# helgeanl/GP-MPC

Measured on NVIDIA H100. Metric: GP predictions/sec (N train x horizon test, fp64), higher is better.
Workload: dtype f64

## Files before the change

gp-mpc_b200/csrc/gpmpc.cu:

```cuda
#include "../../include/gpmpc.h"

#include <dlfcn.h>
#include <math.h>
#include <stdarg.h>
#include <stdlib.h>
#include <string.h>

#include <algorithm>
#include <type_traits>
#include <vector>

#include <nvtx3/nvToolsExt.h>

#include "common.cuh"
#include "gemm_dmma.cuh"
#include "predict_streamk.cuh"
#include "kernels.cuh"

#define GPMPC_VERSION 100
#define HB 64
#define NX_MAX 32
#define PSK_MAX_CTAS 2048
#define MAX_DEPTH 12
#define LOOKAHEAD_MIN_ROWS 1024
// ... 29 lines not shown
        snprintf(err, errn, "libnccl is missing required symbols");
        g_nccl.lib = nullptr;
        return false;
    }
    return true;
}

template <typename T>
struct DevBuf {
    T* p = nullptr;
    size_t cap = 0;
    DevBuf() = default;
    DevBuf(const DevBuf&) = delete;
    DevBuf& operator=(const DevBuf&) = delete;
    ~DevBuf() { cudaFree(p); }
    operator T*() const { return p; }
    int ensure(gpmpc_handle_t h, long long count, const char* name);
};

struct gpmpc_handle_s {
    int N = 0, Nx = 0, Ny = 0, a0 = 0, nloc = 0, Npad = 0, device = 0;
    int nloc_max = 0;
    cudaStream_t st = nullptr;
    cudaEvent_t ev0 = nullptr, ev1 = nullptr;
    cudaStream_t sideSt[MAX_DEPTH] = {nullptr}; cudaEvent_t evA[MAX_DEPTH] = {nullptr}, evB[MAX_DEPTH] = {nullptr}, evT[MAX_DEPTH] = {nullptr}, evS[MAX_DEPTH] = {nullptr};
    long long w2off[MAX_DEPTH + 1] = {0};
    DevBuf<double> dXT, dMu, dY, dHyp, dJit, dHypTmp;
    DevBuf<double> dL, dLi, dW1, dW2;
    DevBuf<double> dAlpha, dTmp, dRes;
    DevBuf<int> dInfo;
    DevBuf<double> dKST, dPart, dPMJ, dSQ, dV, dR, dR2;
    DevBuf<unsigned int> dCnt;
    int psk_ctas = 0, opt_predict_ctas = 0;
    DevBuf<double> dCovV, dCovOut;
    DevBuf<double> dUall, dBeta, dPDV, dPH, dGradOut; bool u_valid = false;
    DevBuf<double> dDR, dVD, dPG, dPB2, dPM3, dHessOut;
    DevBuf<double> dG;
    double *dZ = nullptr, *dSigma = nullptr, *dMean = nullptr, *dVar = nullptr, *dJ = nullptr, *dCov = nullptr;
    DevBuf<double> dRoll;
    DevBuf<double> dIn, dOut;
    int Hcap = 0;
    double* hPinned = nullptr; double* dPinnedAlias = nullptr; size_t hPinnedBytes = 0;
    DevBuf<double> dU, dKinv, dGradPart, dGrad;
    bool has_data = false, has_hyper = false, factorized = false;
    DevBuf<double> dEmTr, dEMP, dEmE, dEmF, dEmW, dEmIJ;
    DevBuf<double> dEmMeanPart, dEmPart, dEmLQ, dEmVec, dEmE2, dEmF2;
    DevBuf<double> dEmKinv, dEmGPart, dEmGRec, dEmBB; bool em_kinv_valid = false;
    std::vector<double> hyper;
    std::vector<double> logdet, yalpha;
    std::vector<int> jitter_used;
    int sms = 132;
    int opt_refine = 0, opt_small_tiles = 528;
    nccl_comm_t comm = nullptr; int rank = 0, world = 1;
    DevBuf<double> dPeerBlock; long long peerGsz = 0; int peerHcap = 0; bool peer_ready = false;
    double* peerBase[GPMPC_MAXW] = {nullptr}; bool peerOpened[GPMPC_MAXW] = {false};
    int* dPeerStatus = nullptr; int* hPeerStatus = nullptr;
    unsigned long long peer_step = 0; int opt_peer = 1; double opt_peer_timeout_s = 60.0; int clock_khz = 1980000;
    char err[512] = "";
};

static void set_error(gpmpc_handle_t h, const char* fmt, ...)
{
    va_list ap; va_start(ap, fmt);
    vsnprintf(h ? h->err : g_create_err, 512, fmt, ap);
    va_end(ap);
}
// ... 198 lines not shown
        const double jit = attempt ? jitter : 0.0;
        CUDA_TRY(cudaMemcpyAsync(h->dJit + a, &jit, sizeof(double), cudaMemcpyHostToDevice, h->st));
        CUDA_TRY(cudaMemsetAsync(h->dInfo + a, 0, sizeof(int), h->st));
        {
            int rck = launch_kbuild(h, dHyp, h->dJit + a, L, 1, 0);
            if (rck) return rck;
        }
        int rc = potrf_inv_rec(h, L, Li, slab(h), slab(h), h->dInfo + a, 0, h->Npad, 1);
        if (rc) return rc;
        int info = 0;
        CUDA_TRY(cudaMemcpyAsync(&info, h->dInfo + a, sizeof(int), cudaMemcpyDeviceToHost, h->st));
        CUDA_TRY(cudaStreamSynchronize(h->st));
        if (info == 0) { *used = attempt; return GPMPC_OK; }
        *used = 1 + info;
    }
    return GPMPC_ERR_NOTPD;
}

extern "C" int gpmpc_version(void) { return GPMPC_VERSION; }

extern "C" const char* gpmpc_last_error(gpmpc_handle_t h) { return h ? h->err : g_create_err; }

extern "C" int gpmpc_destroy(gpmpc_handle_t h);

static int create_fill(gpmpc_handle_t h, int N, int Nx, int Ny, int out_begin, int out_count, int device)
{
    h->N = N; h->Nx = Nx; h->Ny = Ny; h->a0 = out_begin; h->nloc = out_count; h->device = device;
    h->nloc_max = out_count; h->world = 1; h->rank = 0;
    h->Npad = (N + GPMPC_TILE - 1) / GPMPC_TILE * GPMPC_TILE;
    CUDA_TRY(cudaSetDevice(device));
    CUDA_TRY(cudaDeviceGetAttribute(&h->sms, cudaDevAttrMultiProcessorCount, device));
    h->opt_small_tiles = 4 * h->sms;
    h->psk_ctas = PSK_CTAS_PER_SM * h->sms;
    cudaDeviceGetAttribute(&h->clock_khz, cudaDevAttrClockRate, device);
    {
        int lo = 0, hi = 0;
        cudaDeviceGetStreamPriorityRange(&lo, &hi);
        CUDA_TRY(cudaStreamCreateWithPriority(&h->st, cudaStreamNonBlocking, hi));
    }
    CUDA_TRY(cudaEventCreate(&h->ev0));
    CUDA_TRY(cudaEventCreate(&h->ev1));
    const long long np = h->Npad;
    ENSURE(h->dXT, (long long)Nx * np);
    ENSURE(h->dMu, NX_MAX);
    ENSURE(h->dY, (long long)out_count * np);
    ENSURE(h->dHyp, (long long)out_count * (Nx + 2));
    ENSURE(h->dHypTmp, Nx + 2);
    ENSURE(h->dJit, out_count);
    ENSURE(h->dL, out_count * slab(h));
    ENSURE(h->dLi, out_count * slab(h));
    {
        const int nb = h->Npad / 128;
        long long off = 0;
        for (int d = 0; d < MAX_DEPTH; ++d) {
            h->w2off[d] = off;
            const long long nd = (long long)((nb + (1 << d) - 1) >> d) * 128;
            off += nd * nd / 4 + 128;
        }
        h->w2off[MAX_DEPTH] = off;
        int lo = 0, hi = 0;
        cudaDeviceGetStreamPriorityRange(&lo, &hi);
        for (int d = 0; d < MAX_DEPTH; ++d) {
            CUDA_TRY(cudaStreamCreateWithPriority(&h->sideSt[d], cudaStreamNonBlocking, lo));
            CUDA_TRY(cudaEventCreateWithFlags(&h->evA[d], cudaEventDisableTiming));
            CUDA_TRY(cudaEventCreateWithFlags(&h->evB[d], cudaEventDisableTiming));
            CUDA_TRY(cudaEventCreateWithFlags(&h->evT[d], cudaEventDisableTiming));
// ... 291 lines not shown
    if (what == GPMPC_GET_K) return gpmpc_build_K(h, a, dst);
    if (what == GPMPC_GET_ALPHA_NLML) {
        CUDA_TRY(cudaMemcpyAsync(dst, h->dAlpha + (long long)al * h->Npad, h->N * 8, cudaMemcpyDeviceToHost, h->st));
        CUDA_TRY(cudaStreamSynchronize(h->st));
        return GPMPC_OK;
    }
    if (!h->factorized) { set_error(h, "gpmpc_get: call gpmpc_factorize first"); return GPMPC_ERR_STATE; }
    switch (what) {
    case GPMPC_GET_CHOL: return extract_to_host(h, h->dL + (long long)al * slab(h), dst, 1);
    case GPMPC_GET_LINV: return extract_to_host(h, h->dLi + (long long)al * slab(h), dst, 1);
    case GPMPC_GET_ALPHA:
        CUDA_TRY(cudaMemcpyAsync(dst, h->dAlpha + (long long)al * h->Npad, h->N * 8, cudaMemcpyDeviceToHost, h->st));
        CUDA_TRY(cudaStreamSynchronize(h->st));
        return GPMPC_OK;
    case GPMPC_GET_LOGDET: dst[0] = h->logdet[al]; return GPMPC_OK;
    case GPMPC_GET_INVK: {
        int rc = compute_kinv(h, al);
        if (rc) return rc;
        return extract_to_host(h, h->dKinv, dst, 2);
    }
    default: set_error(h, "gpmpc_get: unknown selector %d", what); return GPMPC_ERR_ARG;
    }
}

extern "C" int gpmpc_set_option(gpmpc_handle_t h, const char* name, double value)
{
    if (!h || !name) return GPMPC_ERR_ARG;
    if (!strcmp(name, "refine")) { h->opt_refine = value != 0.0; return GPMPC_OK; }
    if (!strcmp(name, "predict_ctas")) {
        const int v = (int)value;
        if (v < 0 || v > PSK_MAX_CTAS) { set_error(h, "predict_ctas must be in [0, %d]", PSK_MAX_CTAS); return GPMPC_ERR_ARG; }
        h->opt_predict_ctas = v; return GPMPC_OK;
    }
    if (!strcmp(name, "peer_timeout_s")) { h->opt_peer_timeout_s = value > 0.0 ? value : 60.0; return GPMPC_OK; }
    if (!strcmp(name, "small_tiles")) { h->opt_small_tiles = (int)value; return GPMPC_OK; }
    if (!strcmp(name, "peer")) { h->opt_peer = value != 0.0; return GPMPC_OK; }
    set_error(h, "unknown option %s", name);
    return GPMPC_ERR_ARG;
}

static inline int ks_chunk(gpmpc_handle_t h)
{
    if (h->Npad < 8192) return 128;
    return (h->nloc >= 2 && h->Nx <= 12) ? 1024 : 512;
}

static inline int ks_blocks(gpmpc_handle_t h) { return (h->Npad + ks_chunk(h) - 1) / ks_chunk(h); }

static int ensure_rows(gpmpc_handle_t h)
{
    ENSURE(h->dV, (long long)h->nloc * HB * h->Npad);
    ENSURE(h->dR, (long long)h->nloc * HB * h->Npad);
    return GPMPC_OK;
}

static int ensure_predict_bufs(gpmpc_handle_t h, int H)
{
    const long long np = h->Npad, nt = np / 128;
    ENSURE(h->dKST, (long long)h->nloc * HB * np);
    ENSURE(h->dPMJ, (long long)h->nloc * HB * ks_blocks(h) * (h->Nx + 1));
    ENSURE(h->dSQ, (long long)h->nloc * HB * nt);
    ENSURE(h->dCnt, (long long)h->nloc * nt + h->nloc + 1);
    ENSURE(h->dPart, (long long)std::max(h->psk_ctas, h->opt_predict_ctas) * 2 * HB * PSK_BN);
    if (h->opt_refine) {
        int rc = ensure_rows(h);
        if (rc) return rc;
        ENSURE(h->dR2, (long long)h->nloc * HB * np);
    }
    if (H > h->Hcap) {
        h->Hcap = 0;
        h->dZ = h->dSigma = h->dMean = h->dVar = h->dJ = h->dCov = nullptr;
        const long long cap = std::max(H, HB);
        const int nyp = h->nloc_max * h->world;
        const long long Nx = h->Nx, Ny = h->Ny;
        ENSURE(h->dG, (long long)nyp * cap * (Nx + 2));
        ENSURE(h->dIn, cap * Nx + cap * Nx * Nx);
        ENSURE(h->dOut, cap * (2 * Ny + Ny * Nx + Ny * Ny));
        h->dZ = h->dIn; h->dSigma = h->dIn + cap * Nx;
        h->dMean = h->dOut; h->dVar = h->dOut + cap * Ny; h->dJ = h->dOut + 2 * cap * Ny;
        h->dCov = h->dOut + 2 * cap * Ny + cap * Ny * Nx;
        h->Hcap = (int)cap;
    }
    return GPMPC_OK;
}

template <int BM>
static cudaError_t psk_launch_bm(const PredictParams& p, const double* A, long long sA, const double* B, long long sB,
                                 int np, int grid, cudaStream_t st)
{
    constexpr int BYTES = psk_pipe_doubles(BM) * 8 + 2 * PSK_STAGES * 8 + 1024;
    const cudaError_t e = smem_opt_in<predict_streamk_kernel<BM>>(BYTES);
    if (e != cudaSuccess) return e;
    CUtensorMap tmA, tmB;
    if (!tmap_make(&tmA, A, np, BM, np, sA, p.nloc, BM)) return cudaErrorInvalidValue;
    if (!tmap_make(&tmB, B, np, np, np, sB, p.nloc, PSK_BN)) return cudaErrorInvalidValue;
    cudaLaunchConfig_t cfg;
    memset(&cfg, 0, sizeof(cfg));
    cfg.gridDim = dim3(grid); cfg.blockDim = dim3(PSK_THREADS); cfg.dynamicSmemBytes = BYTES; cfg.stream = st;
    cudaLaunchAttribute attr[1];
    attr[0].id = cudaLaunchAttributeProgrammaticStreamSerialization;
    attr[0].val.programmaticStreamSerializationAllowed = 1;
    cfg.attrs = attr; cfg.numAttrs = 1;
    return cudaLaunchKernelEx(&cfg, predict_streamk_kernel<BM>, p, tmA, tmB);
}

static cudaError_t psk_launch(int bm, const PredictParams& p, const double* A, long long sA, const double* B, long long sB,
                              int np, int grid, cudaStream_t st)
{
    switch (bm) {
    case 8: return psk_launch_bm<8>(p, A, sA, B, sB, np, grid, st);
    case 16: return psk_launch_bm<16>(p, A, sA, B, sB, np, grid, st);
    case 24: return psk_launch_bm<24>(p, A, sA, B, sB, np, grid, st);
    case 32: return psk_launch_bm<32>(p, A, sA, B, sB, np, grid, st);
    case 40: return psk_launch_bm<40>(p, A, sA, B, sB, np, grid, st);
    case 48: return psk_launch_bm<48>(p, A, sA, B, sB, np, grid, st);
    case 56: return psk_launch_bm<56>(p, A, sA, B, sB, np, grid, st);
    default: return psk_launch_bm<64>(p, A, sA, B, sB, np, grid, st);
    }
}

static int psk_grid(gpmpc_handle_t h, long long G)
{
    int ctas = h->opt_predict_ctas > 0 ? h->opt_predict_ctas : h->psk_ctas;
    ctas = std::min(ctas, PSK_MAX_CTAS);
    const long long by_work = std::max(1LL, G / 4);
    return (int)std::min<long long>(ctas, h->opt_predict_ctas > 0 ? G : by_work);
}

static void psk_base(gpmpc_handle_t h, PredictParams& p, int Hc, int upper = 0)
{
    memset(&p, 0, sizeof(p));
    const long long nt = h->Npad / 128;
    p.nloc = h->nloc; p.nt = (int)nt; p.Hc = Hc; p.upper = upper;
    p.ntb = (int)((h->Npad + PSK_BN - 1) / PSK_BN); p.nk = h->Npad / GEMM_BK;
    p.T = psk_steps_per_output(p.ntb, p.nk, upper); p.G = p.T * h->nloc;
    p.part = h->dPart;
    p.tile_cnt = h->dCnt; p.out_cnt = h->dCnt + (long long)h->nloc * nt; p.done_cnt = p.out_cnt + h->nloc;
    p.SQ = h->dSQ;
    p.hyp = h->dHyp; p.hyp_ld = h->Nx + 2; p.Nx = h->Nx;
}

static void psk_finalize(gpmpc_handle_t h, PredictParams& p, int H, int h0)
{
    p.finalize = 1; p.PMJ = h->dPMJ; p.nblk_mj = ks_blocks(h);
    p.Gloc = h->dG; p.slot0 = h->a0; p.Htot = H; p.h0 = h0;
}

static AssembleArgs assemble_args(gpmpc_handle_t h, int H, int method, const double* Sigma, int spp,
                                  double* mean, double* var, double* J, double* cov)
{
    AssembleArgs as;
    memset(&as, 0, sizeof(as));
    as.G = h->dG; as.Ny = h->Ny; as.Nx = h->Nx; as.H = H; as.method_ta = (method == GPMPC_METHOD_TA);
    as.Sigma = Sigma; as.sigma_per_point = spp;
    as.mean = mean; as.var = var; as.J = J; as.cov = cov;
    as.world = 1;
    const long long bm1 = (std::min(H, HB) + 7) / 8 * 8;
    as.stage_g = (assemble_rows_doubles(H, h->Ny, h->Nx) <= psk_pipe_doubles((int)bm1)) ? 1 : 0;
    return as;
}

template <int NXP, int CH>
static cudaError_t launch_ks(gpmpc_handle_t h, const double* dZc, int Hc, int bm, int nblk)
{
    const int smem = (NXP + 1) * CH * 8;
    const cudaError_t e = smem_opt_in<ks_tile_kernel<NXP, CH>>(smem);
    if (e != cudaSuccess) return e;
    dim3 g(nblk, bm / 8, h->nloc);
// ... 4 lines not shown

template <int CH>
static cudaError_t launch_ks_nx(gpmpc_handle_t h, const double* dZc, int Hc, int bm, int nblk)
{
    const int Nx = h->Nx;
    if (Nx <= 4) return launch_ks<4, CH>(h, dZc, Hc, bm, nblk);
    if (Nx <= 6) return launch_ks<6, CH>(h, dZc, Hc, bm, nblk);
    if (Nx <= 8) return launch_ks<8, CH>(h, dZc, Hc, bm, nblk);
    if (Nx <= 10) return launch_ks<10, CH>(h, dZc, Hc, bm, nblk);
    if (Nx <= 12) return launch_ks<12, CH>(h, dZc, Hc, bm, nblk);
    if (CH <= 512) {
        if (Nx <= 16) return launch_ks<16, (CH <= 512 ? CH : 512)>(h, dZc, Hc, bm, nblk);
        if (Nx <= 24) return launch_ks<24, (CH <= 512 ? CH : 512)>(h, dZc, Hc, bm, nblk);
        return launch_ks<32, (CH <= 512 ? CH : 512)>(h, dZc, Hc, bm, nblk);
    }
    return cudaErrorInvalidValue;
}

static cudaError_t launch_ks_any(gpmpc_handle_t h, const double* dZc, int Hc, int bm, int nblk)
{
    switch (ks_chunk(h)) {
    case 1024: return launch_ks_nx<1024>(h, dZc, Hc, bm, nblk);
    case 512: return launch_ks_nx<512>(h, dZc, Hc, bm, nblk);
    default: return launch_ks_nx<128>(h, dZc, Hc, bm, nblk);
    }
}

static int tri_product(gpmpc_handle_t h, const double* Amat, const double* T, int bm, int Hc, double* Vout)
{
    const int np = h->Npad;
    PredictParams p;
    psk_base(h, p, Hc);
    p.Vout = Vout; p.sV = (long long)HB * np; p.ldv = np;
    CUDA_TRY(psk_launch(bm, p, Amat, (long long)HB * np, T, slab(h), np, psk_grid(h, p.G), h->st));
    return GPMPC_OK;
}

__global__ void axpby_rows_kernel(const double* __restrict__ x, const double* __restrict__ y, double a, double b,
                                  double* __restrict__ out, long long rowlen, long long srow, int rows)
{
    const long long i = (long long)blockIdx.x * blockDim.x + threadIdx.x;
    const int r = blockIdx.y, bz = blockIdx.z;
    if (i >= rowlen || r >= rows) return;
    const long long o = (long long)bz * srow + (long long)r * rowlen + i;
    out[o] = a * x[o] + b * y[o];
}

static int predict_core(gpmpc_handle_t h, int method, int H, const double* dZ, const double* dSigma, int spp,
                        double* d_mean, double* d_var, double* d_cov, double* d_jac)
{
    const int np = h->Npad, Nx = h->Nx;
    NvtxRange nvtx_r("gpmpc.predict");
    const int use_peers = (h->world > 1 && h->peer_ready && h->opt_peer && H <= h->peerHcap) ? 1 : 0;
    const int nccl_gather = (h->world > 1 && !use_peers) ? 1 : 0;
    const long long timeout_clocks = (long long)(h->opt_peer_timeout_s * 1e3 * (double)h->clock_khz);
    PeerArgs pa;
    memset(&pa, 0, sizeof(pa));
    if (use_peers) {
        h->peer_step += 1;
        for (int r = 0; r < h->world; ++r) pa.base[r] = h->peerBase[r];
        pa.world = h->world; pa.rank = h->rank;
        pa.goff = 2 * GPMPC_MAXW + (long long)(h->peer_step & 1) * h->peerGsz;
        pa.flag_idx = (int)(h->peer_step & 1) * GPMPC_MAXW + h->rank;
        pa.step = h->peer_step;
        pa.timeout_clocks = timeout_clocks;
    }
    AssembleArgs as = assemble_args(h, H, method, dSigma, spp, d_mean, d_var, d_jac, d_cov);
    if (use_peers) as.G = h->dPeerBlock + pa.goff;
    as.flags = use_peers ? reinterpret_cast<const unsigned long long*>(h->dPeerBlock.p) + (h->peer_step & 1) * GPMPC_MAXW : nullptr;
    as.world = h->world; as.step = h->peer_step; as.status = h->dPeerStatus; as.timeout_clocks = timeout_clocks;
    const bool fused_assemble = (H <= HB) && !nccl_gather && ((long long)H * h->Ny * Nx * 8 <= 64 * 1024);
    for (int h0 = 0; h0 < H; h0 += HB) {
        const int Hc = std::min(HB, H - h0);
        const int bm = (Hc + 7) / 8 * 8;
        const bool last_chunk = (h0 + HB >= H);
        const double* dZc = dZ + (long long)h0 * Nx;
        CUDA_TRY(launch_ks_any(h, dZc, Hc, bm, ks_blocks(h)));
        PredictParams p;
        psk_base(h, p, Hc);
        psk_finalize(h, p, H, h0);
        p.pa = pa; p.use_peers = use_peers; p.publish = last_chunk ? 1 : 0;
        p.as = as; p.do_assemble = (fused_assemble && !h->opt_refine) ? 1 : 0;
        if (!h->opt_refine) {
            CUDA_TRY(psk_launch(bm, p, h->dKST, (long long)HB * np, h->dLi, slab(h), np, psk_grid(h, p.G), h->st));
        } else {
            int rc = tri_product(h, h->dKST, h->dLi, bm, Hc, h->dV);
            if (rc) return rc;
            rc = tri_product(h, h->dV, h->dL, bm, Hc, h->dR);
            if (rc) return rc;
            dim3 g((np + 255) / 256, bm, h->nloc);
            axpby_rows_kernel<<<g, 256, 0, h->st>>>(h->dKST, h->dR, 1.0, -1.0, h->dR, np, (long long)HB * np, bm);
            CUDA_TRY(cudaGetLastError());
            rc = tri_product(h, h->dR, h->dLi, bm, Hc, h->dR2);
            if (rc) return rc;
            axpby_rows_kernel<<<g, 256, 0, h->st>>>(h->dV, h->dR2, 1.0, 1.0, h->dV, np, (long long)HB * np, bm);
            CUDA_TRY(cudaGetLastError());
            sq_rows_kernel<<<dim3(np / 128, Hc, h->nloc), 128, 0, h->st>>>(h->dV, np, (long long)HB * np, h->dSQ, np / 128);
            CUDA_TRY(cudaGetLastError());
            finalize_kernel<<<h->nloc, PSK_THREADS, 0, h->st>>>(p);
            CUDA_TRY(cudaGetLastError());
        }
    }
    if (nccl_gather) {
        const size_t cnt = (size_t)h->nloc_max * H * (Nx + 2);
        int r = g_nccl.AllGather(h->dG + (size_t)h->rank * cnt, h->dG, cnt, 8 , h->comm, h->st);
        if (r) { set_error(h, "ncclAllGather failed: %s", g_nccl.GetErrorString ? g_nccl.GetErrorString(r) : "?"); return GPMPC_ERR_NCCL; }
    }
    if (!fused_assemble || h->opt_refine) {
        const int smem = (2 * h->Ny * Nx + h->Ny) * 8;
        assemble_kernel<<<std::min(H, 2048), 128, smem, h->st>>>(as);
        CUDA_TRY(cudaGetLastError());
    }
    return GPMPC_OK;
}

static bool lu_factor(int n, double* A, int* piv, double* det)
{
// ... 643 lines not shown
    }
    const long long per = (long long)Ny * Nx + (long long)Ny * Ny * Nx + (long long)Ny * Nx * Nx;
    ENSURE(h->dGradOut, (long long)std::max(H, HB) * per);
    double* d_dvar = h->dGradOut;
    double* d_dcov = d_dvar + (long long)H * Ny * Nx;
    double* d_hess = d_dcov + (long long)H * Ny * Ny * Nx;
    const long long nxx = (long long)Nx * Nx, ntri = (long long)Nx * (Nx + 1) * (Nx + 2) / 6;
    double *d_d2var = nullptr, *d_d3mean = nullptr, *d_d2cov = nullptr, *d_sh = nullptr;
    if (ho) {
        ENSURE(h->dDR, (long long)h->nloc * HB * np);
        ENSURE(h->dVD, (long long)h->nloc * HB * np);
        ENSURE(h->dPG, (long long)h->nloc * HB * nblk_g * npairs);
        ENSURE(h->dPB2, (long long)h->nloc * HB * nblk_g * npairs);
        ENSURE(h->dPM3, (long long)h->nloc * HB * nblk_g * ntri);
        const long long hper = 2 * Ny * nxx + Ny * nxx * Nx + (long long)Ny * Ny * nxx;
        ENSURE(h->dHessOut, (long long)std::max(H, HB) * hper);
        d_d2var = h->dHessOut;
        d_sh = d_d2var + (long long)H * Ny * nxx;
        d_d3mean = d_sh + (long long)H * Ny * nxx;
        d_d2cov = d_d3mean + (long long)H * Ny * nxx * Nx;
    }
    const size_t nz = (size_t)H * Nx, ns = (method == GPMPC_METHOD_TA) ? (size_t)(spp ? H : 1) * Nx * Nx : 0;
    CUDA_TRY(cudaMemcpyAsync(h->dZ, Z, nz * 8, cudaMemcpyHostToDevice, h->st));
    if (ns) CUDA_TRY(cudaMemcpyAsync(h->dSigma, Sigma, ns * 8, cudaMemcpyHostToDevice, h->st));
    const AssembleArgs as = assemble_args(h, H, method, h->dSigma, spp, h->dMean, h->dVar, h->dJ, h->dCov);
    for (int h0 = 0; h0 < H; h0 += HB) {
        const int Hc = std::min(HB, H - h0), bm = (Hc + 7) / 8 * 8;
        const double* dZc = h->dZ + (long long)h0 * Nx;
        CUDA_TRY(launch_ks_any(h, dZc, Hc, bm, ks_blocks(h)));
        PredictParams p;
        psk_base(h, p, Hc);
        psk_finalize(h, p, H, h0);
        p.Vout = h->dV; p.sV = (long long)HB * np; p.ldv = np;
        CUDA_TRY(psk_launch(bm, p, h->dKST, (long long)HB * np, h->dLi, slab(h), np, psk_grid(h, p.G), h->st));
        psk_base(h, p, Hc, 1);
        p.Vout = h->dBeta; p.sV = (long long)HB * np; p.ldv = np;
        CUDA_TRY(psk_launch(bm, p, h->dV, (long long)HB * np, h->dUall, slab(h), np, psk_grid(h, p.G), h->st));
        CUDA_TRY(nxp_dispatch(Nx, [&](auto nxp) { return launch_grad_reduce<decltype(nxp)::value>(h, dZc, Hc, nblk_g); }));
        grad_finalize_kernel<<<dim3(Hc, h->nloc), 128, 0, h->st>>>(h->dPDV, h->dPH, nblk_g, Hc, h->dHyp, Nx + 2, Nx, Ny,
                                                                   h->dG, H, h0, d_dvar, d_hess);
        CUDA_TRY(cudaGetLastError());
        if (ho) {
            rc = hess_chunk(h, dZc, Hc, H, h0, d_d2var, d_d3mean);
            if (rc) return rc;
        }
    }
    {
        const int smem = (2 * Ny * Nx + Ny) * 8;
        assemble_kernel<<<std::min(H, 2048), 128, smem, h->st>>>(as);
        CUDA_TRY(cudaGetLastError());
        grad_cov_kernel<<<H, 128, 2 * Ny * Nx * 8, h->st>>>(Ny, Nx, method == GPMPC_METHOD_TA, h->dSigma, spp, h->dJ, d_dvar, d_hess, d_dcov);
        CUDA_TRY(cudaGetLastError());
        if (ho) {
            hess_cov_kernel<<<H, 128, 2 * Ny * Nx * 8, h->st>>>(Ny, Nx, method == GPMPC_METHOD_TA, h->dSigma, spp, h->dJ, d_hess,
                                                                d_d2var, d_d3mean, d_sh, d_d2cov);
            CUDA_TRY(cudaGetLastError());
        }
    }
    if (mean) CUDA_TRY(cudaMemcpyAsync(mean, h->dMean, (size_t)H * Ny * 8, cudaMemcpyDeviceToHost, h->st));
    if (var) CUDA_TRY(cudaMemcpyAsync(var, h->dVar, (size_t)H * Ny * 8, cudaMemcpyDeviceToHost, h->st));
    if (cov) CUDA_TRY(cudaMemcpyAsync(cov, h->dCov, (size_t)H * Ny * Ny * 8, cudaMemcpyDeviceToHost, h->st));
    if (jac) CUDA_TRY(cudaMemcpyAsync(jac, h->dJ, (size_t)H * Ny * Nx * 8, cudaMemcpyDeviceToHost, h->st));
    if (dvar_dz) CUDA_TRY(cudaMemcpyAsync(dvar_dz, d_dvar, (size_t)H * Ny * Nx * 8, cudaMemcpyDeviceToHost, h->st));
    if (dcov_dz) CUDA_TRY(cudaMemcpyAsync(dcov_dz, d_dcov, (size_t)H * Ny * Ny * Nx * 8, cudaMemcpyDeviceToHost, h->st));
    if (hess) CUDA_TRY(cudaMemcpyAsync(hess, d_hess, (size_t)H * Ny * Nx * Nx * 8, cudaMemcpyDeviceToHost, h->st));
    if (ho && ho->d2var_dz2) CUDA_TRY(cudaMemcpyAsync(ho->d2var_dz2, d_d2var, (size_t)H * Ny * nxx * 8, cudaMemcpyDeviceToHost, h->st));
    if (ho && ho->d3mean_dz3) CUDA_TRY(cudaMemcpyAsync(ho->d3mean_dz3, d_d3mean, (size_t)H * Ny * nxx * Nx * 8, cudaMemcpyDeviceToHost, h->st));
    if (ho && ho->d2cov_dz2) CUDA_TRY(cudaMemcpyAsync(ho->d2cov_dz2, d_d2cov, (size_t)H * Ny * Ny * nxx * 8, cudaMemcpyDeviceToHost, h->st));
    CUDA_TRY(cudaStreamSynchronize(h->st));
    return GPMPC_OK;
// ... 181 lines not shown
    }
    h->peer_ready = true; h->peer_step = 0;
    return GPMPC_OK;
}

extern "C" int gpmpc_get_size(gpmpc_handle_t h, int* N, int* Nx, int* Ny)
{
    if (!h) return GPMPC_ERR_ARG;
    if (N) *N = h->N;
    if (Nx) *Nx = h->Nx;
    if (Ny) *Ny = h->Ny;
    return GPMPC_OK;
}

extern "C" void* gpmpc_stream(gpmpc_handle_t h) { return h ? (void*)h->st : nullptr; }

extern "C" int gpmpc_synchronize(gpmpc_handle_t h)
{
    if (!h) return GPMPC_ERR_ARG;
    CUDA_TRY(cudaSetDevice(h->device));
    CUDA_TRY(cudaStreamSynchronize(h->st));
    return peer_status_check(h);
}

extern "C" int gpmpc_profile_balance(gpmpc_handle_t h, int H, double* out4)
{
    if (!h || !out4 || H < 1 || H > HB) return GPMPC_ERR_ARG;
    if (!h->factorized) { set_error(h, "gpmpc_profile_balance: call gpmpc_factorize first"); return GPMPC_ERR_STATE; }
    CUDA_TRY(cudaSetDevice(h->device));
    int rc = ensure_predict_bufs(h, HB);
    if (rc) return rc;
    PredictParams p;
    psk_base(h, p, H);
    const int grid = psk_grid(h, p.G);
    DevBuf<unsigned long long> dbg;
    ENSURE(dbg, (long long)grid * 2);
    p.dbg = dbg;
    const int np = h->Npad, bm = (H + 7) / 8 * 8;
    for (int rep = 0; rep < 2; ++rep) {
        cudaError_t e = psk_launch(bm, p, h->dKST, (long long)HB * np, h->dLi, slab(h), np, grid, h->st);
        if (e != cudaSuccess) { set_error(h, "profile_balance: %s", cudaGetErrorString(e)); return GPMPC_ERR_CUDA; }
    }
    std::vector<unsigned long long> t((size_t)grid * 2);
    cudaMemcpyAsync(t.data(), dbg, t.size() * 8, cudaMemcpyDeviceToHost, h->st);
    cudaStreamSynchronize(h->st);
    unsigned long long lo = ~0ull, hi = 0; double mn = 1e300, mx = 0.0, sum = 0.0;
    for (int c = 0; c < grid; ++c) {
        const double d = (double)(t[2 * c + 1] - t[2 * c]) * 1e-3;
        mn = std::min(mn, d); mx = std::max(mx, d); sum += d;
        lo = std::min(lo, t[2 * c]); hi = std::max(hi, t[2 * c + 1]);
    }
    out4[0] = mn; out4[1] = mx; out4[2] = sum / grid; out4[3] = (double)(hi - lo) * 1e-3;
    return GPMPC_OK;
}

extern "C" int gpmpc_profile_tail(gpmpc_handle_t h, int H, double* out8)
{
    if (!h || !out8 || H < 1 || H > HB) return GPMPC_ERR_ARG;
    if (!h->factorized) { set_error(h, "gpmpc_profile_tail: call gpmpc_factorize first"); return GPMPC_ERR_STATE; }
    if (h->world != 1 || h->nloc != h->Ny) { set_error(h, "gpmpc_profile_tail: single-rank handles only"); return GPMPC_ERR_STATE; }
    CUDA_TRY(cudaSetDevice(h->device));
    int rc = ensure_predict_bufs(h, HB);
    if (rc) return rc;
    const int np = h->Npad, bm = (H + 7) / 8 * 8;
    PredictParams p;
    psk_base(h, p, H);
    const int grid = psk_grid(h, p.G);
    DevBuf<unsigned long long> dbg;
    ENSURE(dbg, (long long)grid * 2 + 8);
    p.dbg = dbg;
    psk_finalize(h, p, H, 0);
    p.as = assemble_args(h, H, GPMPC_METHOD_TA, h->dSigma, 0, h->dMean, h->dVar, h->dJ, h->dCov);
    p.as.dbg = dbg + 2 * grid;
    p.do_assemble = 1;
    for (int rep = 0; rep < 2; ++rep) {
        cudaError_t e = psk_launch(bm, p, h->dKST, (long long)HB * np, h->dLi, slab(h), np, grid, h->st);
        if (e != cudaSuccess) { set_error(h, "profile_tail: %s", cudaGetErrorString(e)); return GPMPC_ERR_CUDA; }
    }
    std::vector<unsigned long long> t((size_t)grid * 2 + 8);
    cudaMemcpyAsync(t.data(), dbg, t.size() * 8, cudaMemcpyDeviceToHost, h->st);
    cudaStreamSynchronize(h->st);
    unsigned long long lo = ~0ull, hi = 0, hi2 = 0; int cmax = 0;
    for (int c = 0; c < grid; ++c) {
        lo = std::min(lo, t[2 * c]);
        if (t[2 * c + 1] > hi) { hi2 = hi; hi = t[2 * c + 1]; cmax = c; } else hi2 = std::max(hi2, t[2 * c + 1]);
    }
    for (int k = 0; k < 6; ++k) out8[k] = ((double)t[2 * grid + k] - (double)hi2) * 1e-3;
    out8[6] = (double)(hi - lo) * 1e-3;
    out8[7] = (double)(t[2 * cmax + 1] - t[2 * cmax]) * 1e-3;
    return GPMPC_OK;
}

extern "C" int gpmpc_profile_leaf(gpmpc_handle_t h, double* out15)
{
    if (!h || !out15) return GPMPC_ERR_ARG;
    if (!h->has_data || !h->has_hyper) { set_error(h, "gpmpc_profile_leaf: set_data and set_hyper first"); return GPMPC_ERR_STATE; }
    CUDA_TRY(cudaSetDevice(h->device));
    DevBuf<long long> d;
    ENSURE(d, 16);
    CUDA_TRY(cudaMemcpyToSymbol(d_leaf_prof, &d.p, sizeof(d.p)));
// ... 29 lines not shown
            const int n1 = (nn / 128 / 2) * 128, n2 = nn - n1;
            if (n1 < 128) { set_error(h, "gpmpc_profile: SYRK needs N >= 256"); return GPMPC_ERR_ARG; }
            GemmParams p;
            memset(&p, 0, sizeof(p));
            p.A = h->dW1; p.lda = n1; p.B = h->dW1; p.ldb = n1;
            p.C = h->dLi; p.ldc = np; p.Cin = h->dLi; p.ldcin = np;
            p.mt = n2 / 128; p.nt = n2 / 128; p.K = n1; p.alpha = -1e-30; p.beta = 1.0; p.lower = 1;
            cudaError_t e = gemm128(h, h->st, true, p, 1);
            if (e != cudaSuccess) { set_error(h, "profile syrk: %s", cudaGetErrorString(e)); return GPMPC_ERR_CUDA; }
            return GPMPC_OK;
        }
        case GPMPC_PROF_FACTORIZE: {
            int r = launch_kbuild(h, h->dHyp, h->dJit, h->dL, 1, 0);
            if (r) return r;
            return potrf_inv_rec(h, h->dL, h->dLi, slab(h), slab(h), h->dInfo, 0, np, 1);
        }
        case GPMPC_PROF_TRIGEMM: {
            const int Hc = (n > 0 && n <= HB) ? n : 56;
            return tri_product(h, h->dKST, h->dLi, (Hc + 7) / 8 * 8, Hc, nullptr);
        }
        case GPMPC_PROF_KS: {
            const int Hc = (n > 0 && n <= HB) ? n : 56;
            cudaError_t e = launch_ks_any(h, h->dZ, Hc, (Hc + 7) / 8 * 8, ks_blocks(h));
            if (e != cudaSuccess) { set_error(h, "profile ks: %s", cudaGetErrorString(e)); return GPMPC_ERR_CUDA; }
            return GPMPC_OK;
        }
        case GPMPC_PROF_PREDICT_TAIL: {
            const int Hc = (n > 0 && n <= HB) ? n : 56;
            PredictParams p;
            psk_base(h, p, Hc);
            psk_finalize(h, p, Hc, 0);
            p.as = assemble_args(h, Hc, GPMPC_METHOD_TA, h->dSigma, 0, h->dMean, h->dVar, h->dJ, h->dCov);
            p.do_assemble = (h->world == 1 && h->nloc == h->Ny) ? 1 : 0;
            cudaError_t e = psk_launch((Hc + 7) / 8 * 8, p, h->dKST, (long long)HB * np, h->dLi, slab(h), np, psk_grid(h, p.G), h->st);
            if (e != cudaSuccess) { set_error(h, "profile predict tail: %s", cudaGetErrorString(e)); return GPMPC_ERR_CUDA; }
            return GPMPC_OK;
        }
        default: set_error(h, "gpmpc_profile: unknown selector %d", what); return GPMPC_ERR_ARG;
        }
    };
    if (what == GPMPC_PROF_TRIGEMM || what == GPMPC_PROF_KS || what == GPMPC_PROF_PREDICT_TAIL) { rc = ensure_predict_bufs(h, HB); if (rc) return rc; }
    CUDA_TRY(cudaMemsetAsync(h->dJit, 0, h->nloc * sizeof(double), h->st));
    rc = run();
    if (rc) return rc;
    CUDA_TRY(cudaStreamSynchronize(h->st));
    CUDA_TRY(cudaEventRecord(h->ev0, h->st));
    for (int r = 0; r < reps; ++r) { rc = run(); if (rc) return rc; }
    CUDA_TRY(cudaEventRecord(h->ev1, h->st));
    CUDA_TRY(cudaEventSynchronize(h->ev1));
    CUDA_TRY(cudaEventElapsedTime(&ms, h->ev0, h->ev1));
    ms_out[0] = (double)ms / reps;
    if (what != GPMPC_PROF_TRIGEMM && what != GPMPC_PROF_KS && what != GPMPC_PROF_PREDICT_TAIL) h->factorized = false;
    return GPMPC_OK;
}
```

gp-mpc_b200/csrc/predict_streamk.cuh:

```cuda
#pragma once
#include "common.cuh"
#include "gemm_dmma.cuh"

#define GPMPC_MAXW 16
#define PSK_CW 8
#define PSK_BN (32 * PSK_CW)
#define PSK_STAGES 5
#define PSK_CTAS_PER_SM 1
#define PSK_THREADS (32 * PSK_CW)

__host__ __device__ constexpr long long psk_pipe_doubles(int bm) { return (long long)PSK_STAGES * (bm + PSK_BN) * GEMM_BK; }


struct PeerArgs {
    double* base[GPMPC_MAXW];
    int world, rank;
    long long goff;
    int flag_idx;
    unsigned long long step;
    long long timeout_clocks;
};

struct AssembleArgs {
    const double* G;
    int Ny, Nx, H, method_ta;
    const double* Sigma; int sigma_per_point;
    double *mean, *var, *J, *cov;
    const unsigned long long* flags;
    int world; unsigned long long step; int* status;
    long long timeout_clocks;
    unsigned long long* dbg;
    int stage_g;
};

struct PredictParams {
    int nloc, nt, Hc;
    int ntb, nk;
    int upper;
    long long T, G;
    double* part;
    unsigned int* tile_cnt;
    unsigned int* out_cnt;
    unsigned int* done_cnt;
    double* SQ;
    double* Vout; long long sV; int ldv;
    int finalize;
    const double* PMJ; int nblk_mj;
    const double* hyp; int hyp_ld, Nx;
    double* Gloc; int slot0, Htot, h0;
    PeerArgs pa; int use_peers, publish;
    AssembleArgs as; int do_assemble;
    unsigned long long* dbg;
};

__device__ __forceinline__ void tail_stamp(unsigned long long* dbg, int k, int tid)
{
    if (dbg && tid == 0) { unsigned long long t; asm volatile("mov.u64 %0, %%globaltimer;" : "=l"(t)); dbg[k] = t; }
}

template <bool WARP>
__device__ __forceinline__ void assemble_point(const AssembleArgs& A, int h, double* sh, int tid, int nth)
{
    const int Ny = A.Ny, Nx = A.Nx, H = A.H;
    double* Jh = sh; double* JS = sh + Ny * Nx; double* vh = sh + 2 * Ny * Nx;
    for (int idx = tid; idx < Ny * Nx; idx += nth) {
        const int a = idx / Nx, d = idx % Nx;
        const double v = __ldcg(A.G + (((long long)a) * H + h) * (Nx + 2) + 2 + d);
        Jh[idx] = v;
        if (A.J) A.J[((long long)h * Ny + a) * Nx + d] = v;
    }
    for (int a = tid; a < Ny; a += nth) {
        const double* g = A.G + (((long long)a) * H + h) * (Nx + 2);
// ... 176 lines not shown
                *reinterpret_cast<volatile int*>(A.status) = 1 + tid;
                *reinterpret_cast<volatile int*>(sh_ok) = 0;
                break;
            }
            __nanosleep(64);
        } while (true);
    }
    __syncthreads();
    return *reinterpret_cast<volatile int*>(sh_ok) != 0;
}

__global__ void __launch_bounds__(128)
assemble_kernel(const AssembleArgs A)
{
    extern __shared__ double sh[];
    __shared__ int ok;
    if (!peer_acquire(A, threadIdx.x, &ok)) return;
    for (int h = blockIdx.x; h < A.H; h += gridDim.x) assemble_point<false>(A, h, sh, threadIdx.x, blockDim.x);
}

#define PSK_SB (PSK_BN / GEMM_BK)
__host__ __device__ inline long long psk_kstart(int ntb, int nk, int upper, int jt)
{
    const long long full = (long long)(PSK_SB / 2) * jt * (jt + 1), d = (long long)PSK_SB * ntb - nk;
    return upper ? full - jt * d : (jt == ntb ? full - d : full);
}
__host__ __device__ inline long long psk_steps_per_output(int ntb, int nk, int upper) { return psk_kstart(ntb, nk, upper, ntb); }
__device__ __forceinline__ long long psk_kstart(const PredictParams& p, int jt) { return psk_kstart(p.ntb, p.nk, p.upper, jt); }
__device__ __forceinline__ int psk_ksteps(const PredictParams& p, int jt)
{
    return p.upper ? p.nk - PSK_SB * (p.ntb - 1 - jt) : min(PSK_SB * (jt + 1), p.nk);
}

struct PskIter { int a, jt, s, ks; };

__device__ __forceinline__ void psk_iter_init(PskIter& it, long long g, const PredictParams& p)
{
    it.a = (int)(g / p.T);
    const long long r = g - (long long)it.a * p.T;
    int jt = (int)((sqrt(8.0 * (double)r / PSK_SB + 1.0) - 1.0) * 0.5);
    jt = max(0, min(jt, p.ntb - 1));
    while (jt > 0 && psk_kstart(p, jt) > r) --jt;
    while (jt + 1 < p.ntb && psk_kstart(p, jt + 1) <= r) ++jt;
    it.jt = jt; it.s = (int)(r - psk_kstart(p, jt)); it.ks = psk_ksteps(p, jt);
}
__device__ __forceinline__ void psk_iter_next(PskIter& it, const PredictParams& p)
{
    if (++it.s == it.ks) {
        it.s = 0;
        if (++it.jt == p.ntb) { it.jt = 0; ++it.a; }
        it.ks = psk_ksteps(p, it.jt);
    }
}

__device__ __forceinline__ void psk_store_record(const PredictParams& p, int a, int h, int q, double val)
{
    const long long off = (((long long)(p.slot0 + a)) * p.Htot + p.h0 + h) * (p.Nx + 2) + q;
    if (!p.use_peers) p.Gloc[off] = val;
    else for (int r = 0; r < p.pa.world; ++r) p.pa.base[r][p.pa.goff + off] = val;
}

__device__ __forceinline__ void psk_reduce_mj(const PredictParams& p, int i_begin, int i_end, int t, int nthr)
{
    const int F1 = p.Nx + 1;
    for (int i = i_begin + t; i < i_end; i += nthr) {
        const int ah = i / F1, qq = i - ah * F1, a = ah / p.Hc, h = ah - a * p.Hc;
// ... 85 lines not shown
    extern __shared__ double sh[];
    __shared__ unsigned int s_flag;
    __shared__ int s_ok;
    const int per = p.Hc * (p.Nx + 1);
    psk_reduce_mj(p, blockIdx.x * per, (blockIdx.x + 1) * per, threadIdx.x, PSK_THREADS);
    psk_finalize_output(p, blockIdx.x, threadIdx.x, PSK_THREADS);
    psk_step_tail(p, sh, threadIdx.x, PSK_THREADS, &s_flag, &s_ok);
}

template <int BM>
__global__ void __launch_bounds__(PSK_THREADS, PSK_CTAS_PER_SM)
predict_streamk_kernel(const PredictParams p, const __grid_constant__ CUtensorMap tmA, const __grid_constant__ CUtensorMap tmB)
{
    constexpr int BK = GEMM_BK, BN = PSK_BN, STAGES = PSK_STAGES, CW = PSK_CW, NT = PSK_THREADS;
    constexpr int NF = BM / 8;
    static_assert(BK == 16 && BN == 32 * CW && BN % 128 == 0, "one m16n8k16 per fragment and k-step, 32 L-rows per warp");
    constexpr int GR = BN / 128;
    constexpr int A_STAGE = BM * BK, B_STAGE = BN * BK;
    constexpr uint32_t STAGE_TX = (BM + BN) * BK * 8;
    static_assert(BM % 8 == 0 && BM >= 8 && BM <= 64, "BM");

    extern __shared__ __align__(16) double smem_raw[];
    double* smem = smem_align1024(smem_raw);
    double* As = smem;
    double* Bs = smem + STAGES * A_STAGE;
    uint64_t* full = reinterpret_cast<uint64_t*>(smem + STAGES * (A_STAGE + B_STAGE));
    uint64_t* empty = full + STAGES;
    __shared__ double red[BN / 16][64];
    __shared__ unsigned int s_flag;
    __shared__ int s_ok;

    const int tid = threadIdx.x, warp = tid >> 5, lane = tid & 31, g = lane >> 2, t = lane & 3;
    const long long C = gridDim.x, c = blockIdx.x;
    const long long g0 = p.G * c / C;
    const int nsteps = (int)(p.G * (c + 1) / C - g0);
    if (nsteps <= 0) return;
    if (p.dbg && threadIdx.x == 0) { unsigned long long t0; asm volatile("mov.u64 %0, %%globaltimer;" : "=l"(t0)); p.dbg[2 * blockIdx.x] = t0; }

    __shared__ PskIter s_pit;
    __shared__ int s_pg;
    __shared__ uint64_t s_pol[2];
    if (tid == 0) {
#pragma unroll
        for (int s = 0; s < STAGES; ++s) { mbar_init(full + s, 1); mbar_init(empty + s, CW); }
        mbar_fence_init();
    }
    __syncthreads();

    auto issue = [&]() {
        PskIter it = s_pit;
        const int pg = s_pg, s = pg % STAGES;
        if (pg >= STAGES) mbar_wait(empty + s, (uint32_t)(((pg / STAGES) - 1) & 1));
        mbar_arrive_expect_tx(full + s, STAGE_TX);
        const int jta = p.upper ? p.ntb - 1 - it.jt : it.jt;
        const int k0 = (p.upper ? jta * BN : 0) + it.s * BK;
        tma_tile_g2s_3d_hint(As + s * A_STAGE, &tmA, k0, 0, it.a, full + s, s_pol[1]);
        tma_tile_g2s_3d_hint(Bs + s * B_STAGE, &tmB, k0, jta * BN, it.a, full + s, s_pol[0]);
        psk_iter_next(it, p);
        s_pit = it;
        s_pg = pg + 1;
    };
    constexpr int AHEAD = STAGES - 2;
    asm volatile("griddepcontrol.wait;" ::: "memory");
    if (tid == 0) {
        PskIter it;
        psk_iter_init(it, g0, p);
        s_pit = it; s_pg = 0;
        s_pol[0] = l2_policy_evict_first(); s_pol[1] = l2_policy_evict_last();
#pragma unroll
        for (int s = 0; s < AHEAD; ++s)
            if (s_pg < nsteps) issue();
    }
    if (p.finalize) {
        const int tot = p.nloc * p.Hc * (p.Nx + 1), per = (tot + (int)C - 1) / (int)C;
        if (tid >= 32) {
            psk_reduce_mj(p, min(tot, (int)c * per), min(tot, ((int)c + 1) * per), tid - 32, NT - 32);
            if (p.use_peers) __threadfence_system();
        }
    }

    PskIter cit;
    psk_iter_init(cit, g0, p);
    int cj[4];
#pragma unroll
    for (int j = 0; j < 4; ++j) cj[j] = (((j + 4 * (t >> 1)) ^ g) << 1) + (t & 1);
    int i = 0;
    while (i < nsteps) {
        const int a = cit.a, jt = cit.jt, s_begin = cit.s, ksteps = cit.ks;
        const int seg = min(ksteps - s_begin, nsteps - i);
        const int hh = warp / (128 / 32);
        const int st_lo = p.upper ? (128 / BK) * hh : 0;
        const int st_hi = p.upper ? ksteps : PSK_SB * jt + (128 / BK) * (hh + 1);
        double acc[2][NF][4];
#pragma unroll
        for (int mi = 0; mi < 2; ++mi)
#pragma unroll
            for (int ni = 0; ni < NF; ++ni)
#pragma unroll
                for (int r = 0; r < 4; ++r) acc[mi][ni][r] = 0.0;

        for (int q = 0; q < seg; ++q, ++i) {
            const int s = i % STAGES;
            if (tid == 0 && i + AHEAD < nsteps) issue();
            mbar_wait(full + s, (uint32_t)((i / STAGES) & 1));
            const int st = s_begin + q;
            if (st >= st_lo && st < st_hi) {
                const double* ls = Bs + s * B_STAGE + (warp * 32 + g) * 16;
                const double* ps = As + s * A_STAGE + g * 16;
                double av[2][8];
#pragma unroll
                for (int mi = 0; mi < 2; ++mi)
#pragma unroll
                    for (int j = 0; j < 4; ++j) { av[mi][2 * j] = ls[256 * mi + cj[j]]; av[mi][2 * j + 1] = ls[256 * mi + 128 + cj[j]]; }
#pragma unroll
                for (int ni = 0; ni < NF; ++ni) {
                    double bv[4];
#pragma unroll
                    for (int j = 0; j < 4; ++j) bv[j] = ps[ni * 8 * 16 + cj[j]];
                    dmma16816(acc[0][ni], av[0], bv);
                    dmma16816(acc[1][ni], av[1], bv);
                }
            }
            __syncwarp();
            if (lane == 0) mbar_arrive(empty + s);
        }
        cit.s = s_begin + seg - 1;
        psk_iter_next(cit, p);

        bool have_tile = true;
        if (seg != ksteps) {
            const long long tg0 = (long long)a * p.T + psk_kstart(p, jt), tg1 = tg0 + ksteps;
            const long long Cf = gridDim.x;
            const int c_first = (int)(((tg0 + 1) * Cf - 1) / p.G), c_last = (int)((tg1 * Cf - 1) / p.G);
            double2* mine = reinterpret_cast<double2*>(p.part + ((long long)blockIdx.x * 2 + (s_begin == 0 ? 1 : 0)) * (BM * BN)) + tid;
#pragma unroll
            for (int mi = 0; mi < 2; ++mi)
#pragma unroll
                for (int ni = 0; ni < NF; ++ni)
#pragma unroll
                    for (int hf = 0; hf < 2; ++hf)
                        __stcg(mine + ((mi * NF + ni) * 2 + hf) * NT, make_double2(acc[mi][ni][2 * hf], acc[mi][ni][2 * hf + 1]));
            __threadfence();
            __syncthreads();
            if (tid == 0) {
                unsigned int* cnt = p.tile_cnt + (long long)a * p.ntb + jt;
                const unsigned int old = atomicAdd(cnt, 1u);
                const unsigned int last = (old == (unsigned int)(c_last - c_first)) ? 1u : 0u;
                if (last) *cnt = 0u;
                s_flag = last;
            }
            __syncthreads();
            have_tile = s_flag != 0u;
            if (have_tile) {
                __threadfence();
#pragma unroll
                for (int mi = 0; mi < 2; ++mi)
#pragma unroll
                    for (int ni = 0; ni < NF; ++ni)
#pragma unroll
                        for (int r = 0; r < 4; ++r) acc[mi][ni][r] = 0.0;
                for (int cc = c_first; cc <= c_last; ++cc) {
                    const double2* src = reinterpret_cast<const double2*>(p.part + ((long long)cc * 2 + (cc == c_first ? 1 : 0)) * (BM * BN)) + tid;
#pragma unroll
                    for (int mi = 0; mi < 2; ++mi)
#pragma unroll
                        for (int ni = 0; ni < NF; ++ni)
#pragma unroll
                            for (int hf = 0; hf < 2; ++hf) {
                                const double2 v = __ldcg(src + ((mi * NF + ni) * 2 + hf) * NT);
                                acc[mi][ni][2 * hf] += v.x; acc[mi][ni][2 * hf + 1] += v.y;
                            }
                }
            }
        }
        if (!have_tile) continue;

        const int jta = p.upper ? p.ntb - 1 - jt : jt;
        const int row0 = jta * BN + warp * 32;
        if (p.Vout && row0 < p.nk * BK) {
            double* vo = p.Vout + (long long)a * p.sV + row0 + g;
#pragma unroll
            for (int mi = 0; mi < 2; ++mi)
#pragma unroll
                for (int ni = 0; ni < NF; ++ni)
#pragma unroll
                    for (int r = 0; r < 4; ++r)
                        vo[(long long)(ni * 8 + 2 * t + (r & 1)) * p.ldv + 16 * mi + 8 * (r >> 1)] = acc[mi][ni][r];
        }
#pragma unroll
        for (int mi = 0; mi < 2; ++mi)
#pragma unroll
            for (int ni = 0; ni < NF; ++ni)
#pragma unroll
                for (int j = 0; j < 2; ++j) {
                    double r = acc[mi][ni][j] * acc[mi][ni][j];
// ... 37 lines not shown
```

Measured before the change: 14240.

## Split stream-K predict work into L2-sized rounds of outputs

Partitions the stream-K predict work into rounds, each covering as many outputs as fit in half the L2 cache. Every CTA takes a slice of every round, so at any moment all CTAs work on the same small set of output B-matrices and keep them resident in L2. The partial-sum buffer grows by the number of rounds, and the fixup indexing becomes per-round. When the outputs are few or small, the single round behaves as before, apart from extra index arithmetic.

```diff
diff --git a/gp-mpc_b200/csrc/gpmpc.cu b/gp-mpc_b200/csrc/gpmpc.cu
--- a/gp-mpc_b200/csrc/gpmpc.cu
+++ b/gp-mpc_b200/csrc/gpmpc.cu
@@ -85,6 +85,7 @@
     DevBuf<double> dKST, dPart, dPMJ, dSQ, dV, dR, dR2;
     DevBuf<unsigned int> dCnt;
     int psk_ctas = 0, opt_predict_ctas = 0;
+    int l2_bytes = 0, opt_round_outputs = 0;
     DevBuf<double> dCovV, dCovOut;
     DevBuf<double> dUall, dBeta, dPDV, dPH, dGradOut; bool u_valid = false;
     DevBuf<double> dDR, dVD, dPG, dPB2, dPM3, dHessOut;
@@ -349,6 +350,7 @@
     CUDA_TRY(cudaDeviceGetAttribute(&h->sms, cudaDevAttrMultiProcessorCount, device));
     h->opt_small_tiles = 4 * h->sms;
     h->psk_ctas = PSK_CTAS_PER_SM * h->sms;
+    CUDA_TRY(cudaDeviceGetAttribute(&h->l2_bytes, cudaDevAttrL2CacheSize, device));
     cudaDeviceGetAttribute(&h->clock_khz, cudaDevAttrClockRate, device);
     {
         int lo = 0, hi = 0;
@@ -706,6 +708,11 @@
         if (v < 0 || v > PSK_MAX_CTAS) { set_error(h, "predict_ctas must be in [0, %d]", PSK_MAX_CTAS); return GPMPC_ERR_ARG; }
         h->opt_predict_ctas = v; return GPMPC_OK;
     }
+    if (!strcmp(name, "predict_round_outputs")) {
+        const int v = (int)value;
+        if (v < 0) { set_error(h, "predict_round_outputs must be >= 0"); return GPMPC_ERR_ARG; }
+        h->opt_round_outputs = v; return GPMPC_OK;
+    }
     if (!strcmp(name, "peer_timeout_s")) { h->opt_peer_timeout_s = value > 0.0 ? value : 60.0; return GPMPC_OK; }
     if (!strcmp(name, "small_tiles")) { h->opt_small_tiles = (int)value; return GPMPC_OK; }
     if (!strcmp(name, "peer")) { h->opt_peer = value != 0.0; return GPMPC_OK; }
@@ -728,6 +735,14 @@
     return GPMPC_OK;
 }
 
+#define PSK_L2_SHARE 0.5
+static int psk_round_outputs(gpmpc_handle_t h)
+{
+    if (h->opt_round_outputs > 0) return std::min(h->opt_round_outputs, h->nloc);
+    const long long fit = (long long)(PSK_L2_SHARE * h->l2_bytes) / ((long long)HB * h->Npad * 8);
+    return (int)std::max(1LL, std::min<long long>(fit, h->nloc));
+}
+
 static int ensure_predict_bufs(gpmpc_handle_t h, int H)
 {
     const long long np = h->Npad, nt = np / 128;
@@ -735,7 +750,8 @@
     ENSURE(h->dPMJ, (long long)h->nloc * HB * ks_blocks(h) * (h->Nx + 1));
     ENSURE(h->dSQ, (long long)h->nloc * HB * nt);
     ENSURE(h->dCnt, (long long)h->nloc * nt + h->nloc + 1);
-    ENSURE(h->dPart, (long long)std::max(h->psk_ctas, h->opt_predict_ctas) * 2 * HB * PSK_BN);
+    const int R = psk_round_outputs(h), rounds = (h->nloc + R - 1) / R;
+    ENSURE(h->dPart, (long long)std::max(h->psk_ctas, h->opt_predict_ctas) * rounds * 2 * HB * PSK_BN);
     if (h->opt_refine) {
         int rc = ensure_rows(h);
         if (rc) return rc;
@@ -793,12 +809,13 @@
     }
 }
 
-static int psk_grid(gpmpc_handle_t h, long long G)
+static int psk_grid(gpmpc_handle_t h, const PredictParams& p)
 {
     int ctas = h->opt_predict_ctas > 0 ? h->opt_predict_ctas : h->psk_ctas;
     ctas = std::min(ctas, PSK_MAX_CTAS);
-    const long long by_work = std::max(1LL, G / 4);
-    return (int)std::min<long long>(ctas, h->opt_predict_ctas > 0 ? G : by_work);
+    const long long Gmin = psk_round_steps(p, psk_rounds(p) - 1);
+    const long long by_work = std::max(1LL, Gmin / 4);
+    return (int)std::min<long long>(ctas, h->opt_predict_ctas > 0 ? Gmin : by_work);
 }
 
 static void psk_base(gpmpc_handle_t h, PredictParams& p, int Hc, int upper = 0)
@@ -808,6 +825,7 @@
     p.nloc = h->nloc; p.nt = (int)nt; p.Hc = Hc; p.upper = upper;
     p.ntb = (int)((h->Npad + PSK_BN - 1) / PSK_BN); p.nk = h->Npad / GEMM_BK;
     p.T = psk_steps_per_output(p.ntb, p.nk, upper); p.G = p.T * h->nloc;
+    p.R = psk_round_outputs(h);
     p.part = h->dPart;
     p.tile_cnt = h->dCnt; p.out_cnt = h->dCnt + (long long)h->nloc * nt; p.done_cnt = p.out_cnt + h->nloc;
     p.SQ = h->dSQ;
@@ -878,7 +896,7 @@
     PredictParams p;
     psk_base(h, p, Hc);
     p.Vout = Vout; p.sV = (long long)HB * np; p.ldv = np;
-    CUDA_TRY(psk_launch(bm, p, Amat, (long long)HB * np, T, slab(h), np, psk_grid(h, p.G), h->st));
+    CUDA_TRY(psk_launch(bm, p, Amat, (long long)HB * np, T, slab(h), np, psk_grid(h, p), h->st));
     return GPMPC_OK;
 }
 
@@ -928,7 +946,7 @@
         p.pa = pa; p.use_peers = use_peers; p.publish = last_chunk ? 1 : 0;
         p.as = as; p.do_assemble = (fused_assemble && !h->opt_refine) ? 1 : 0;
         if (!h->opt_refine) {
-            CUDA_TRY(psk_launch(bm, p, h->dKST, (long long)HB * np, h->dLi, slab(h), np, psk_grid(h, p.G), h->st));
+            CUDA_TRY(psk_launch(bm, p, h->dKST, (long long)HB * np, h->dLi, slab(h), np, psk_grid(h, p), h->st));
         } else {
             int rc = tri_product(h, h->dKST, h->dLi, bm, Hc, h->dV);
             if (rc) return rc;
@@ -1638,10 +1656,10 @@
         psk_base(h, p, Hc);
         psk_finalize(h, p, H, h0);
         p.Vout = h->dV; p.sV = (long long)HB * np; p.ldv = np;
-        CUDA_TRY(psk_launch(bm, p, h->dKST, (long long)HB * np, h->dLi, slab(h), np, psk_grid(h, p.G), h->st));
+        CUDA_TRY(psk_launch(bm, p, h->dKST, (long long)HB * np, h->dLi, slab(h), np, psk_grid(h, p), h->st));
         psk_base(h, p, Hc, 1);
         p.Vout = h->dBeta; p.sV = (long long)HB * np; p.ldv = np;
-        CUDA_TRY(psk_launch(bm, p, h->dV, (long long)HB * np, h->dUall, slab(h), np, psk_grid(h, p.G), h->st));
+        CUDA_TRY(psk_launch(bm, p, h->dV, (long long)HB * np, h->dUall, slab(h), np, psk_grid(h, p), h->st));
         CUDA_TRY(nxp_dispatch(Nx, [&](auto nxp) { return launch_grad_reduce<decltype(nxp)::value>(h, dZc, Hc, nblk_g); }));
         grad_finalize_kernel<<<dim3(Hc, h->nloc), 128, 0, h->st>>>(h->dPDV, h->dPH, nblk_g, Hc, h->dHyp, Nx + 2, Nx, Ny,
                                                                    h->dG, H, h0, d_dvar, d_hess);
@@ -1889,7 +1907,7 @@
     if (rc) return rc;
     PredictParams p;
     psk_base(h, p, H);
-    const int grid = psk_grid(h, p.G);
+    const int grid = psk_grid(h, p);
     DevBuf<unsigned long long> dbg;
     ENSURE(dbg, (long long)grid * 2);
     p.dbg = dbg;
@@ -1922,7 +1940,7 @@
     const int np = h->Npad, bm = (H + 7) / 8 * 8;
     PredictParams p;
     psk_base(h, p, H);
-    const int grid = psk_grid(h, p.G);
+    const int grid = psk_grid(h, p);
     DevBuf<unsigned long long> dbg;
     ENSURE(dbg, (long long)grid * 2 + 8);
     p.dbg = dbg;
@@ -2018,7 +2036,7 @@
             psk_finalize(h, p, Hc, 0);
             p.as = assemble_args(h, Hc, GPMPC_METHOD_TA, h->dSigma, 0, h->dMean, h->dVar, h->dJ, h->dCov);
             p.do_assemble = (h->world == 1 && h->nloc == h->Ny) ? 1 : 0;
-            cudaError_t e = psk_launch((Hc + 7) / 8 * 8, p, h->dKST, (long long)HB * np, h->dLi, slab(h), np, psk_grid(h, p.G), h->st);
+            cudaError_t e = psk_launch((Hc + 7) / 8 * 8, p, h->dKST, (long long)HB * np, h->dLi, slab(h), np, psk_grid(h, p), h->st);
             if (e != cudaSuccess) { set_error(h, "profile predict tail: %s", cudaGetErrorString(e)); return GPMPC_ERR_CUDA; }
             return GPMPC_OK;
         }
diff --git a/gp-mpc_b200/csrc/predict_streamk.cuh b/gp-mpc_b200/csrc/predict_streamk.cuh
--- a/gp-mpc_b200/csrc/predict_streamk.cuh
+++ b/gp-mpc_b200/csrc/predict_streamk.cuh
@@ -38,6 +38,7 @@
     int ntb, nk;
     int upper;
     long long T, G;
+    int R;
     double* part;
     unsigned int* tile_cnt;
     unsigned int* out_cnt;
@@ -280,6 +281,29 @@
     return p.upper ? p.nk - PSK_SB * (p.ntb - 1 - jt) : min(PSK_SB * (jt + 1), p.nk);
 }
 
+__host__ __device__ inline int psk_rounds(const PredictParams& p) { return (p.nloc + p.R - 1) / p.R; }
+__host__ __device__ inline long long psk_round_steps(const PredictParams& p, int r)
+{
+    return (long long)(p.nloc - r * p.R < p.R ? p.nloc - r * p.R : p.R) * p.T;
+}
+__host__ __device__ inline void psk_round_range(const PredictParams& p, int r, long long c, long long C, long long& g0, long long& g1)
+{
+    const long long off = (long long)r * p.R * p.T, Gr = psk_round_steps(p, r);
+    g0 = off + Gr * c / C; g1 = off + Gr * (c + 1) / C;
+}
+
+__device__ __forceinline__ int psk_next_round(const PredictParams& p, int r, long long c, long long C, long long& g0, int& n)
+{
+    const int nr = psk_rounds(p);
+    for (++r; r < nr; ++r) {
+        long long g1;
+        psk_round_range(p, r, c, C, g0, g1);
+        n = (int)(g1 - g0);
+        if (n > 0) break;
+    }
+    return r;
+}
+
 struct PskIter { int a, jt, s, ks; };
 
 __device__ __forceinline__ void psk_iter_init(PskIter& it, long long g, const PredictParams& p)
@@ -431,13 +455,15 @@
 
     const int tid = threadIdx.x, warp = tid >> 5, lane = tid & 31, g = lane >> 2, t = lane & 3;
     const long long C = gridDim.x, c = blockIdx.x;
-    const long long g0 = p.G * c / C;
-    const int nsteps = (int)(p.G * (c + 1) / C - g0);
+    long long g0;
+    int n0, nsteps = 0;
+    const int r0 = psk_next_round(p, -1, c, C, g0, n0);
+    for (int r = psk_rounds(p) - 1; r >= r0; --r) { long long r_lo, r_hi; psk_round_range(p, r, c, C, r_lo, r_hi); nsteps += (int)(r_hi - r_lo); }
     if (nsteps <= 0) return;
     if (p.dbg && threadIdx.x == 0) { unsigned long long t0; asm volatile("mov.u64 %0, %%globaltimer;" : "=l"(t0)); p.dbg[2 * blockIdx.x] = t0; }
 
     __shared__ PskIter s_pit;
-    __shared__ int s_pg;
+    __shared__ int s_pg, s_pr, s_pleft;
     __shared__ uint64_t s_pol[2];
     if (tid == 0) {
 #pragma unroll
@@ -456,6 +482,12 @@
         tma_tile_g2s_3d_hint(As + s * A_STAGE, &tmA, k0, 0, it.a, full + s, s_pol[1]);
         tma_tile_g2s_3d_hint(Bs + s * B_STAGE, &tmB, k0, jta * BN, it.a, full + s, s_pol[0]);
         psk_iter_next(it, p);
+        if (--s_pleft == 0) {
+            long long gn;
+            int nn;
+            s_pr = psk_next_round(p, s_pr, blockIdx.x, gridDim.x, gn, nn);
+            if (s_pr < psk_rounds(p)) { psk_iter_init(it, gn, p); s_pleft = nn; }
+        }
         s_pit = it;
         s_pg = pg + 1;
     };
@@ -464,7 +496,7 @@
     if (tid == 0) {
         PskIter it;
         psk_iter_init(it, g0, p);
-        s_pit = it; s_pg = 0;
+        s_pit = it; s_pg = 0; s_pr = r0; s_pleft = n0;
         s_pol[0] = l2_policy_evict_first(); s_pol[1] = l2_policy_evict_last();
 #pragma unroll
         for (int s = 0; s < AHEAD; ++s)
@@ -486,7 +518,11 @@
     int i = 0;
     while (i < nsteps) {
         const int a = cit.a, jt = cit.jt, s_begin = cit.s, ksteps = cit.ks;
-        const int seg = min(ksteps - s_begin, nsteps - i);
+        long long r_lo, r_hi;
+        psk_round_range(p, a / p.R, blockIdx.x, gridDim.x, r_lo, r_hi);
+        const long long r_left = r_hi - ((long long)a * p.T + psk_kstart(p, jt) + s_begin);
+        const bool round_end = r_left <= ksteps - s_begin;
+        const int seg = round_end ? (int)r_left : ksteps - s_begin;
         const int hh = warp / (128 / 32);
         const int st_lo = p.upper ? (128 / BK) * hh : 0;
         const int st_hi = p.upper ? ksteps : PSK_SB * jt + (128 / BK) * (hh + 1);
@@ -525,13 +561,20 @@
         }
         cit.s = s_begin + seg - 1;
         psk_iter_next(cit, p);
+        if (round_end && i < nsteps) {
+            long long gn;
+            int nn;
+            psk_next_round(p, a / p.R, blockIdx.x, gridDim.x, gn, nn);
+            psk_iter_init(cit, gn, p);
+        }
 
         bool have_tile = true;
         if (seg != ksteps) {
-            const long long tg0 = (long long)a * p.T + psk_kstart(p, jt), tg1 = tg0 + ksteps;
+            const int r = a / p.R, nr = psk_rounds(p);
+            const long long tg0 = (long long)(a - r * p.R) * p.T + psk_kstart(p, jt), tg1 = tg0 + ksteps, Gr = psk_round_steps(p, r);
             const long long Cf = gridDim.x;
-            const int c_first = (int)(((tg0 + 1) * Cf - 1) / p.G), c_last = (int)((tg1 * Cf - 1) / p.G);
-            double2* mine = reinterpret_cast<double2*>(p.part + ((long long)blockIdx.x * 2 + (s_begin == 0 ? 1 : 0)) * (BM * BN)) + tid;
+            const int c_first = (int)(((tg0 + 1) * Cf - 1) / Gr), c_last = (int)((tg1 * Cf - 1) / Gr);
+            double2* mine = reinterpret_cast<double2*>(p.part + (((long long)blockIdx.x * nr + r) * 2 + (s_begin == 0 ? 1 : 0)) * (BM * BN)) + tid;
 #pragma unroll
             for (int mi = 0; mi < 2; ++mi)
 #pragma unroll
@@ -559,7 +602,7 @@
 #pragma unroll
                         for (int r = 0; r < 4; ++r) acc[mi][ni][r] = 0.0;
                 for (int cc = c_first; cc <= c_last; ++cc) {
-                    const double2* src = reinterpret_cast<const double2*>(p.part + ((long long)cc * 2 + (cc == c_first ? 1 : 0)) * (BM * BN)) + tid;
+                    const double2* src = reinterpret_cast<const double2*>(p.part + (((long long)cc * nr + r) * 2 + (cc == c_first ? 1 : 0)) * (BM * BN)) + tid;
 #pragma unroll
                     for (int mi = 0; mi < 2; ++mi)
 #pragma unroll
```

Result: no change. 14320 (median of 6 runs) (+0.6%).
